# atoms-ufrj/atomsmm

Measured on AMD Instinct MI355X. Metric: ns/day on 100k-atom TIP3P RESPA box; near-nonbonded HBM GB/s vs 8 TB/s peak, higher is better.
Workload: dtype f64

## Files before the change

atomsmm_amd/csrc/abi.hip:

```cpp
#include <algorithm>
#include <cmath>
#include <cstring>
#include <numeric>

#include "amm_ctx.h"
#include "cluster.h"

int amm_pair_setup_grid(amm_ctx *ctx, PairForce *pf);
static bool amm_family_allows_cluster(int family, int flags) {
    const bool tab_family = family == AMM_NEAR_NONE || family == AMM_NEAR_SHIFT || family == AMM_NEAR_FSWITCH || family == AMM_DAMPED || family == AMM_NONBONDED;
    return tab_family && !(flags & (AMM_GROUP_LJ | AMM_GROUP_Q));
}
int amm_bonded_arity(int kind);
int amm_bonded_npar(int kind);

static thread_local std::string g_error;
void amm_set_error(const std::string &msg) { g_error = msg; }

static PairForce *get_pair(amm_ctx *ctx, int id) {
    if (!ctx || id < 0 || id >= (int)ctx->forces.size() || ctx->forces[id].type != AMM_FORCE_PAIR) {
        amm_set_error("invalid pair force id");
        return nullptr;
    }
    return ctx->forces[id].pair;
// ... 1208 lines not shown
    PairForce *pf = get_pair(ctx, force_id);
    if (!pf || !d_pos || !count) {
        amm_set_error("amm_pair_count_within: null argument or not a pair force");
        return 1;
    }
    if (pf->free_space) {
        amm_set_error("amm_pair_count_within: a free-space pair force (AMM_FREE_SPACE) has no neighbour rows to count");
        return 1;
    }
    long long c = 0;
    PairForce *Lw = pf->host ? pf->host : pf;
    if (Lw->last_kind >= 1 && Lw->cl && Lw->cl->built) {
        if (amm_cluster_count_within_impl(ctx, pf, d_pos, r_within, &c)) return 1;
        if (Lw->last_kind == 2 && pf->rest && Lw->rest && Lw->rest->built) {
            long long c2 = 0;
            if (amm_pair_count_within_impl(ctx, pf->rest, d_pos, r_within, &c2)) return 1;
            c += c2;
        }
    } else if (amm_pair_count_within_impl(ctx, pf, d_pos, r_within, &c)) return 1;
    *count = (int64_t)c;
    return 0;
}

const char *amm_kernel_revision(void) { return amm_kernel_revision_impl(); }

int amm_set_outer_skin(amm_ctx *ctx, double skin_out) {
    ctx->skin_out = skin_out;
    return 0;
}

int amm_set_option(amm_ctx *ctx, const char *name, double value) {
    if (!ctx || !name) {
        amm_set_error("amm_set_option: null argument");
        return 1;
    }
    const std::string k(name);
    const int v = (int)value;
    if (k == "cluster") ctx->opt_cluster = v;
    else if (k == "hybrid") ctx->opt_hybrid = v;
    else if (k == "small_group") ctx->opt_small_group = v;
    else if (k == "mixed_terms") ctx->opt_mixed_terms = v;
    else if (k == "rest_skin_factor") ctx->opt_rest_skin_factor = value;
    else if (k == "tab") ctx->opt_tab = v;
    else if (k == "site_trips") ctx->site_trips = v != 0;
    else if (k == "lanes_per_row") ctx->opt_lpa = v;
    else if (k == "build_parts") ctx->opt_parts = v;
    else if (k == "build_split") ctx->opt_build_split = v;
    else if (k == "unroll") ctx->opt_unroll = v;
    else if (k == "dual_unroll") ctx->opt_dual_unroll = v;
    else if (k == "tab_block") ctx->opt_tab_bs = v;
    else if (k == "tab_dual_block") ctx->opt_tab_dual_bs = v;
    else if (k == "fuse_rows") ctx->opt_fuse_rows = v;
    else if (k == "row_phases") ctx->opt_row_phases = v;
    else if (k == "group_candidates") ctx->opt_group_candidates = v;
    else if (k == "positions_private") ctx->opt_positions_private = v;
    else if (k == "site_tab") ctx->opt_site_tab = v;
    else if (k == "terms_from") ctx->opt_terms_from = v;
    else if (k == "no_term_lanes") ctx->opt_no_term_lanes = v;
    else if (k == "fuse_epilogue") ctx->opt_fuse_epilogue = v;
    else if (k == "comm_timeout") ctx->opt_comm_timeout = value;
    else if (k == "spec_assign") ctx->opt_spec_assign = v;
    else if (k == "chargeless") ctx->opt_chargeless = v;
    else if (k == "state_exchange") ctx->opt_state_exchange = v;
    else {
        amm_set_error("amm_set_option: unknown option '" + k + "'");
        return 1;
    }
    return 0;
}

static const double AMM_BOX_SKIN_KEEP = 0.5;
static const double AMM_BOX_ROWS_GROW = 1.25;

static double grid_room(const amm_ctx *ctx, const CellGrid &g) {
    double room = 1.0e30;
    for (int k = 0; k < 3; ++k) room = std::min(room, 2.0 * ctx->box.L[k] / g.nc[k]);
    return room;
}
static bool grid_differs(const amm_ctx *ctx, const CellGrid &g, double reach) {
    for (int k = 0; k < 3; ++k) {
        int nc = (int)floor(ctx->box.L[k] / (0.5 * reach));
        nc = std::max(1, std::min(512, nc));
        if (nc != g.nc[k]) return true;
    }
    return false;
}
static bool box_within(const amm_ctx *ctx, const double L0[3], double tol) {
    for (int k = 0; k < 3; ++k)
        if (std::fabs(ctx->box.L[k] - L0[k]) > tol * L0[k]) return false;
    return true;
}

static int box_apply(amm_ctx *ctx, bool &regrid, bool &waited) {
    const double V = ctx->box.L[0] * ctx->box.L[1] * ctx->box.L[2];
    for (auto &fo : ctx->forces) {
        if (fo.type != AMM_FORCE_PAIR || fo.pair->free_space) continue;
        PairForce *pf = fo.pair;
        pair_derive_buffers(ctx, pf);
        if (pf->rest) pf->rest->skin_req = pf->skin * ctx->opt_rest_skin_factor;
    }
    auto wait_once = [&]() -> int {
        if (!waited) AMM_HIP(hipStreamSynchronize(ctx->stream));
        waited = true;
        return 0;
    };
    for (auto &fo : ctx->forces) {
// ... 202 lines not shown
```

atomsmm_amd/csrc/amm_ctx.h:

```cpp
#pragma once
#include <hip/hip_runtime.h>

#include <cstdint>
#include <string>
#include <vector>

#include "../../include/atomsmm_hip.h"

#define AMM_WAVE 64
#define AMM_MAX_PRE 6
#define AMM_DERIV_LAMBDA 1024
#define AMM_MAX_GROUPS 33

void amm_set_error(const std::string &msg);
#define AMM_HIP(call)                                                                            \
    do {                                                                                         \
        hipError_t e_ = (call);                                                                  \
        if (e_ != hipSuccess) {                                                                  \
            amm_set_error(std::string(#call) + ": " + hipGetErrorString(e_));                    \
            return 1;                                                                            \
        }                                                                                        \
    } while (0)

struct PairTab {
// ... 244 lines not shown
#define AMM_MAX_WATCH 4
struct ListWatch {
    const double *xref = nullptr;
    double thr2 = 0;
    int *flags = nullptr;
    long *pre_epoch = nullptr;
    const double **pre_pos = nullptr;
};

static inline int amm_slice_per(int n, int world) {
    const int nc = (n + 2) / 3;
    return 3 * ((nc + world - 1) / world);
}

struct EpiPlan {
    BondedSet *bs = nullptr;
    double *f0 = nullptr;
    int npre = 0, niter = 0;
    const double *pre_a[AMM_MAX_PRE] = {nullptr}, *pre_b[AMM_MAX_PRE] = {nullptr};
    double pre_coef[AMM_MAX_PRE] = {0};
    int pre_plus[AMM_MAX_PRE] = {0};
    double c1 = 0, d = 0, c2 = 0;
    PairForce *next = nullptr;
    int kind = 0;
    int with_move = 0;
    double dcoef = 0;
};

struct amm_ctx {
    int n = 0;
    int opt_spec_assign = 1;
    int opt_state_exchange = 1;
    int opt_chargeless = 1;
    int opt_fuse_epilogue = 1;
    const EpiPlan *epi_request = nullptr;
    bool epi_done = false;
    long long n_epilogues = 0;
    long long n_state_exchanges = 0;
    std::vector<const double *> own_only;
    long long n_copies_current = 0;
    int opt_cluster = 1;
    int opt_hybrid = 1;
    double opt_rest_skin_factor = 2.0;
    int opt_mixed_terms = 1;
    int opt_small_group = 1;
    bool creating_rest = false;
    int opt_tab = 1;
    int opt_build_split = 0;
    int opt_lpa = 0, opt_parts = 0, opt_unroll = 2, opt_dual_unroll = 2, opt_tab_bs = 0, opt_tab_dual_bs = 0;
    int opt_site_tab = 1;
    CZeroRows zero_rows = CZeroRows{0, nullptr, nullptr, nullptr};
    int opt_positions_private = 0;
    int opt_group_candidates = 1;
    int opt_row_phases = 1;
    int opt_fuse_rows = 1;
    int opt_terms_from = 8192, opt_no_term_lanes = 0;
    ListWatch watched[AMM_MAX_WATCH];
    int n_watched = 0;
    int device = 0;
    hipStream_t stream = nullptr;
    Box box;
    bool has_box = true;
    int rank = 0, world = 1;
    std::vector<ForceObj> forces;
    double *d_x = nullptr, *d_v = nullptr;
    const double *d_mass = nullptr;
    double *slots[AMM_MAX_SLOTS] = {nullptr};
    GroupDef groups[AMM_MAX_GROUPS];
    bool profile = false;
    int profile_only = -1;
    double *d_scratch = nullptr;
    double *d_expr_part = nullptr;
    double *d_fscratch = nullptr;
    ConstraintSet *constraints = nullptr;
    std::vector<MinObj *> minimizers;
    std::vector<ExprDef> exprs;
    std::vector<BathDef> baths;
    IsoDef iso;
    RegDef reg;
    unsigned long long expr_seed = 0, expr_counter = 0;
    double *alt_x = nullptr, *alt_v = nullptr, *alt_f = nullptr;
    bool fuse_inner = true;
    bool site_trips = true;
    long long box_changes = 0, box_regrids = 0, box_waits = 0;
    int n_mol = 0, n_mol_small = 0, n_mol_long = 0;
    int *d_mol_ptr = nullptr, *d_mol_atoms = nullptr, *d_mol_small = nullptr, *d_mol_long = nullptr;
    long pos_epoch = 0;
    double skin_out = -1.0;
    void *comm = nullptr;
    bool comm_failed = false;
    double opt_comm_timeout = 0;
    double *d_xchg = nullptr;
    long long xchg_doubles = 0;
    PendingExchange pending;
    long long comm_calls = 0, comm_doubles = 0;
};

struct KickList {
    const double *f[4], *f2[4];
    int plus[4];
    double coef[4];
    int n;
};

#define AMM_FLAG_FAR 12
struct WatchArgs {
// ... 95 lines not shown
```

atomsmm_amd/csrc/cluster.hip:

```cpp
#include <algorithm>
#include <cmath>
#include <cstdio>
#include <cstdlib>
#include <cstring>
#include <type_traits>
#include <vector>

#include "amm_ctx.h"
#include "bonded_terms.h"
#include "cluster.h"
#include "device_utils.h"
#include "pair_math.h"
#include "pair_tab.h"

#ifndef AMM_EXP_NOLJ
#define AMM_EXP_NOLJ 0
#endif

__device__ double amm_erfcx_table_dev_c[AMM_ERFCX_NI * AMM_ERFCX_NC];
static bool g_erfcx_uploaded_c[64] = {false};

void amm_cluster_classify(int n, const std::vector<int> &ptr, const std::vector<int> &idx, std::vector<int> &mol_first, std::vector<int> &rest) {
    mol_first.clear();
    rest.clear();
// ... 828 lines not shown
                    }
                    row_cnt = lane == t ? (nf | (nb_ << 16)) : row_cnt;
                    j0 += nch;
                }
                CBS_STAMP(5);
                __syncthreads();
                CBS_STAMP(6);
            }
            if (w == 0 && lane < nt) {
                const int count = row_cnt & 0xffff, countf = (int)((unsigned)row_cnt >> 16);
                const int total_nb = count + countf;
                const bool over = total_nb > cap;
                nnb[tb + lane - c_begin] = over ? 0 : total_nb;
                nnb_near[tb + lane - c_begin] = over ? 0 : count;
                if (over) flags[1] = 1;
                wsum += (unsigned long long)total_nb;
                wnear += (unsigned long long)count;
                wmax = max(wmax, total_nb);
            }
        }
    }
    __syncthreads();
    }
    for (int off = 32; off > 0; off >>= 1) {
        wsum += __shfl_xor(wsum, off);
        wnear += __shfl_xor(wnear, off);
        wmax = max(wmax, __shfl_xor(wmax, off));
    }
    if (w == 0 && lane == 0) {
        amm_st_l2(&blockstats[3 * blockIdx.x], wsum);
        amm_st_l2(&blockstats[3 * blockIdx.x + 1], (unsigned long long)wmax);
        amm_st_l2(&blockstats[3 * blockIdx.x + 2], wnear);
    }
    if (amm_last_block(ticket)) cfinish_build_block(flags, counters, blockstats, (int)gridDim.x, 0);
}

#define AMM_CPHASES 6
struct CPairArgs {
    int c_begin, nrows, lpa_shift, cap;
    const int *aperm;
    const int *nl, *nnb, *nnb_total;
    const double4 *posq;
    const double2 *lj;
    double *force;
    int accumulate, sorted_out;
    Box box;
    const double *host_tab;
    int host_bytes;
    double margin;
    int ntask;
    int per_pair_image;
    int rpx, nphase;
    int ph_off[AMM_CPHASES], ph_shift[AMM_CPHASES], ph_ntask[AMM_CPHASES];
#ifdef AMM_CPAIR_TIMING
    unsigned long long *wave_times;
#endif
    const double *host_tab_ss;
    int host_ss_bytes, host_ss_off, site_atoms;
    double hsig_site, seps2_site;
    const double *guest_tab, *guest_tab_ss;
    int guest_bytes, guest_ss_bytes, guest_ss_off, g_accumulate;
    const double *tab_image;
    unsigned long long host_serial, guest_serial;
    PairForce *tab_owner;
    double *gforce;
    double gfac, gsr;
};

#ifdef AMM_CPAIR_TIMING
#define CWALK_T_PARAM , unsigned long long &t_first
#define CWALK_T_ARG , t_first
#else
#define CWALK_T_PARAM
#define CWALK_T_ARG
#endif
template <int FAM, int CMODE, int GFAM, int IMG, int SMASK>
__device__ __forceinline__ void cwalk_rows(const CPairArgs &A, const PairConsts &c, const PairConsts &g, const char *tabh, const char *tabg,
                                           const double *erfcx, const double4 (&pi)[3], const double2 *li, int i_sites, const int (&so)[3],
                                           const int (&sog)[3], double sign_lj, const int *row, int nfront, int nn, int sub, int lpa,
                                           int self, double (&f)[9], double (&fg)[9] CWALK_T_PARAM) {
    constexpr bool DUAL = GFAM >= 0;
    constexpr bool SS = SMASK != 0;
    const int back = A.cap - 1 + nfront;
    const double r2low = DUAL ? fmax(c.tab.r2min, g.tab.r2min) : c.tab.r2min;
    const double r2low_ss = DUAL ? fmax(c.tab.ss_r2min, g.tab.ss_r2min) : c.tab.ss_r2min;
    auto entry = [&](int k) { return k < nn ? row[k < nfront ? k : back - k] : self; };
    auto load_pos = [&](int e, int b) {
        return *reinterpret_cast<const double4 *>(reinterpret_cast<const char *>(A.posq) + (size_t)((unsigned)e & 0x1fffffffu) * 96u + 32 * b);
    };
    auto load_lj = [&](int e, int b) {
        double2 l = make_double2(0.0, 0.0);
        if (i_sites != 0 && __builtin_amdgcn_ballot_w64((((unsigned)e >> 29) >> b) & 1u) != 0ull)
            l = *reinterpret_cast<const double2 *>(reinterpret_cast<const char *>(A.lj) + (size_t)((unsigned)e & 0x1fffffffu) * 48u + 16 * b);
        return l;
    };
    double4 pj[3];
    double2 lj[3];
    int k = sub;
    int e = entry(k), en = entry(k + lpa);
#pragma unroll
    for (int b = 0; b < 3; ++b) {
        pj[b] = load_pos(e, b);
        if (!SS) lj[b] = load_lj(e, b);
    }
    while (__builtin_amdgcn_ballot_w64(k < nn) != 0ull) {
        const bool ok = k < nn;
        const bool front = k < nfront;
        const bool any_front = DUAL && __builtin_amdgcn_ballot_w64(front) != 0ull;
        const unsigned bits = (unsigned)e >> 29;
        const int e2 = entry(k + 2 * lpa);
        double sx = 0.0, sy = 0.0, sz = 0.0;
        if (IMG == 1) {
            sx = A.box.L[0] * rint((pj[0].x - pi[0].x) * A.box.invL[0]);
            sy = A.box.L[1] * rint((pj[0].y - pi[0].y) * A.box.invL[1]);
            sz = A.box.L[2] * rint((pj[0].z - pi[0].z) * A.box.invL[2]);
        }
#pragma unroll
        for (int b = 0; b < 3; ++b) {
            const double xb = pj[b].x - sx, yb = pj[b].y - sy, zb = pj[b].z - sz, qb = pj[b].w;
            const int mb = SS ? -(int)((bits >> b) & 1u) : 0;
// ... 402 lines not shown
    return all_most;
}

#ifndef AMM_CBS_SINGLE
#define AMM_CBS_SINGLE 512
#endif

#ifndef AMM_CBS_NEAR
#define AMM_CBS_NEAR 512
#endif
#ifndef AMM_CTAB_WAVES_PER_EU
#define AMM_CTAB_WAVES_PER_EU 1
#endif
template <int FAM, int CMODE, int GFAM, int BS, int SMASK, bool EPI = false>
__global__ void __launch_bounds__(BS) __attribute__((amdgpu_waves_per_eu(AMM_CTAB_WAVES_PER_EU)))
k_cpair(CPairArgs A, PairConsts c, PairConsts g, CEpiArgs E) {
    constexpr bool DUAL = GFAM >= 0;
    constexpr bool SS = SMASK != 0;
    extern __shared__ __align__(16) char s_lds[];
    if (EPI && E.spec_clear) {
        for (int cidx = blockIdx.x * BS + threadIdx.x; cidx <= E.grid.ncell; cidx += gridDim.x * BS) E.spec_clear[cidx] = 0;
    }
#ifdef AMM_CPAIR_TIMING
    const unsigned long long t_entry = wall_clock64();
    unsigned long long t_staged = 0, t_first = 0;
    int n_tasks_done = 0, n_interior = 0;
    unsigned long long t_epi[3] = {0, 0, 0};
#endif
    constexpr int WPB = BS / 64;
    const int lane = threadIdx.x & 63;
    const double sign = c.sign;
    const int xcd = blockIdx.x & 7, nwx = (gridDim.x >> 3) * WPB;
    const int row_end = min((xcd + 1) * A.rpx, A.nrows);
#ifdef AMM_CPAIR_SWAP
    const int wave = (int)(threadIdx.x >> 6) ^ 4;
#else
    const int wave = (int)(threadIdx.x >> 6);
#endif
    const int task0 = (int)(blockIdx.x >> 3) * WPB + __builtin_amdgcn_readfirstlane(wave);
    int phase = 0, task = task0;
    auto seek = [&]() {
        while (phase < A.nphase && task >= A.ph_ntask[phase]) {
            ++phase;
            task = task0;
        }
        return phase < A.nphase;
    };
    constexpr bool AHEAD = SS;
    int shift = 0, lpa = 1, sub = 0, a = 0, cs = 0, nfront = 0, nn = 0;
    bool valid = false;
    const int *row = nullptr;
    double4 pi[3];
    double2 pl[3];
    auto pre_rows = [&]() {
        shift = A.ph_shift[phase];
        lpa = 1 << shift;
        sub = lane & (lpa - 1);
        a = xcd * A.rpx + A.ph_off[phase] + task * (64 >> shift) + (lane >> shift);
        valid = a < row_end;
        cs = A.c_begin + (valid ? a : 0);
#pragma unroll
        for (int t = 0; t < 3; ++t) {
            pi[t] = A.posq[3 * cs + t];
            pl[t] = A.lj[3 * cs + t];
        }
        nfront = valid ? A.nnb[a] : 0;
        nn = valid ? (A.nnb_total ? A.nnb_total[a] : nfront) : 0;
        row = A.nl + (size_t)(valid ? a : 0) * A.cap;
    };
    bool has = seek();
    if (AHEAD && has) pre_rows();

    const int used = A.host_bytes + (DUAL ? A.guest_bytes : 0) + (SS ? A.host_ss_bytes + (DUAL ? A.guest_ss_bytes : 0) : 0);
    double2 tabs[(160 * 1024) / (BS * 16)];
    amm_stage_issue<BS>(tabs, A.tab_image, used);
    amm_stage_commit<BS>(tabs, s_lds, used);
    amm_stage_rest<BS>(tabs, A.tab_image, s_lds, used);
#if defined(AMM_EXP_TAB_GLOBAL)
    const char *tabh = reinterpret_cast<const char *>(A.host_tab);
#else
    const char *tabh = s_lds;
#endif
    const char *tabg = s_lds + A.host_bytes;
    const double *erfcx = amm_erfcx_table_dev_c;
    double2 *s_li = nullptr;
    if (!SS) {
        double *s_erfcx = reinterpret_cast<double *>(s_lds + used);
        for (int k = threadIdx.x; k < AMM_ERFCX_NI * AMM_ERFCX_NC; k += BS) s_erfcx[k] = amm_erfcx_table_dev_c[k];
        erfcx = s_erfcx;
        s_li = reinterpret_cast<double2 *>(s_erfcx + AMM_ERFCX_NI * AMM_ERFCX_NC) + (threadIdx.x >> 6) * 192;
    }
    __syncthreads();
#ifdef AMM_CPAIR_TIMING
    t_staged = wall_clock64();
#endif

    PairConsts c1 = c, g1 = g;
    c1.sign = 1.0;
    g1.sign = 1.0;
    while (has) {
        if (!AHEAD) pre_rows();
        const int t_a = a, t_cs = cs, t_sub = sub, t_lpa = lpa;
        const bool t_valid = valid;
        int i_sites = 0;
        int so[3] = {0, 0, 0}, sog[3] = {0, 0, 0};
        if (!SS) __builtin_amdgcn_wave_barrier();
#pragma unroll
        for (int t = 0; t < 3; ++t) {
            pi[t].w *= c.Kc * sign;
            double2 l = pl[t];
            l.y *= sign;
            if (!SS) s_li[64 * t + lane] = l;
            const bool site = valid && l.y != 0.0;
            if ((SMASK >> t) & 1) {
                so[t] = site ? A.host_ss_off : 0;
                if (DUAL) sog[t] = site ? A.guest_ss_off : 0;
            }
            if (__builtin_amdgcn_ballot_w64(site) != 0ull) i_sites |= 1 << t;
        }
        if (!SS) {
            __builtin_amdgcn_fence(__ATOMIC_RELEASE, "wavefront");
            __builtin_amdgcn_wave_barrier();
            __builtin_amdgcn_fence(__ATOMIC_ACQUIRE, "wavefront");
        }
        const double2 *li = SS ? nullptr : s_li + lane;
        const bool edge = valid && !(pi[0].x >= A.margin && pi[0].x <= A.box.L[0] - A.margin && pi[0].y >= A.margin &&
                                     pi[0].y <= A.box.L[1] - A.margin && pi[0].z >= A.margin && pi[0].z <= A.box.L[2] - A.margin);
        const bool interior = __builtin_amdgcn_ballot_w64(edge) == 0ull;
#ifdef AMM_CPAIR_TIMING
        ++n_tasks_done;
        n_interior += interior ? 1 : 0;
#endif
        double f[9], fg[9];
#pragma unroll
        for (int k = 0; k < 9; ++k) f[k] = fg[k] = 0.0;
        if (A.per_pair_image) cwalk_rows<FAM, CMODE, GFAM, 2, SMASK>(A, c1, g1, tabh, tabg, erfcx, pi, li, i_sites, so, sog, sign, row, nfront, nn, sub, lpa, cs, f, fg CWALK_T_ARG);
        else if (interior) cwalk_rows<FAM, CMODE, GFAM, 0, SMASK>(A, c1, g1, tabh, tabg, erfcx, pi, li, i_sites, so, sog, sign, row, nfront, nn, sub, lpa, cs, f, fg CWALK_T_ARG);
        else cwalk_rows<FAM, CMODE, GFAM, 1, SMASK>(A, c1, g1, tabh, tabg, erfcx, pi, li, i_sites, so, sog, sign, row, nfront, nn, sub, lpa, cs, f, fg CWALK_T_ARG);
        task += nwx;
        has = seek();
        if (AHEAD && has) pre_rows();
        for (int off = t_lpa >> 1; off > 0; off >>= 1) {
#pragma unroll
            for (int k = 0; k < 9; ++k) {
                f[k] += __shfl_xor(f[k], off);
                if (DUAL) fg[k] += __shfl_xor(fg[k], off);
            }
        }
        if (t_valid && t_sub == 0) {
#pragma unroll
            for (int t = 0; t < 3; ++t) {
                const int i = A.sorted_out ? 3 * t_a + t : A.aperm[3 * t_cs + t];
#pragma unroll
                for (int d = 0; d < 3; ++d) {
                    if (A.accumulate) A.force[3 * i + d] += f[3 * t + d];
                    else A.force[3 * i + d] = f[3 * t + d];
                    if (DUAL) {
                        if (A.g_accumulate) A.gforce[3 * i + d] += fg[3 * t + d];
                        else A.gforce[3 * i + d] = fg[3 * t + d];
                    }
                }
            }
        }
    }
#ifdef AMM_CPAIR_TIMING
    if (EPI) t_staged = wall_clock64();
#endif
    if (EPI) {
        for (int phase = 0; phase < A.nphase; ++phase) {
            const int shift = A.ph_shift[phase], row0 = xcd * A.rpx + A.ph_off[phase], ntask = A.ph_ntask[phase];
            const int rpw = 64 >> shift;
            for (int task = (int)(blockIdx.x >> 3) * WPB + (int)(threadIdx.x >> 6); task < ntask; task += nwx) {
                const int a = row0 + task * rpw + (lane >> shift);
                const bool valid = a < row_end;
#ifdef AMM_CPAIR_TIMING
                cepi_rows(E, A.box, A.c_begin + (valid ? a : 0), valid, lane & ((1 << shift) - 1), t_epi);
#else
                cepi_rows(E, A.box, A.c_begin + (valid ? a : 0), valid, lane & ((1 << shift) - 1));
#endif
            }
        }
        if (E.spec_count && amm_last_block(E.spec_ticket)) {
            if (amm_ld_l2(&E.spec_flags[0])) {
                const int fullest = cscan_counts<BS>(E.grid.ncell, E.spec_count, E.spec_start);
                if (threadIdx.x == 0) E.spec_flags[6] = fullest;
            }
        }
    }
#ifdef AMM_CPAIR_TIMING
    if (A.wave_times && (threadIdx.x & 63) == 0) {
        unsigned long long *o = A.wave_times + 4 * ((size_t)blockIdx.x * (BS / 64) + (threadIdx.x >> 6));
        o[0] = t_entry;
        o[1] = t_staged;
        o[2] = wall_clock64();
        o[3] = EPI ? (((t_epi[0] - t_staged) & 0xfffffull) | (((t_epi[1] - t_staged) & 0xfffffull) << 20) | (((t_epi[2] - t_staged) & 0xfffffull) << 40))
                   : ((((t_first ? t_first - t_entry : 0ull) & 0xfffffull) << 24) | ((unsigned long long)(n_interior & 0xffff) << 8) | (unsigned long long)(n_tasks_done & 0xff));
    }
#endif
}

static const double AMM_PHASE_COST[7] = {0, 0, 1.0, 0.55, 0.32, 0.18, 0.11};
static double cpair_plan_rec(int rows, int waves, int s, int off, CPairArgs *P) {
    const int rpw = 64 >> s, per_round = waves * rpw;
    const int full = rows / per_round, left = rows - full * per_round;
    const double finish = (double)((rows + per_round - 1) / per_round) * AMM_PHASE_COST[s];
    auto put = [&](int ntask) {
        if (P && ntask > 0) {
            P->ph_off[P->nphase] = off;
            P->ph_shift[P->nphase] = s;
            P->ph_ntask[P->nphase] = ntask;
            ++P->nphase;
        }
    };
    int s2 = 6;
    double split = 1e300;
    for (int t = s + 1; t <= 6 && left > 0; ++t) {
        const double v = cpair_plan_rec(left, waves, t, 0, nullptr);
        if (v < split) {
            split = v;
            s2 = t;
        }
    }
    split += full * AMM_PHASE_COST[s];
    if (left == 0 || s == 6 || finish <= split) {
        put((rows + rpw - 1) / rpw);
        return finish;
    }
    put(full * waves);
    cpair_plan_rec(left, waves, s2, off + full * per_round, P);
    return split;
}
static void cpair_plan(CPairArgs &P, int waves, int enabled) {
    P.rpx = (P.nrows + 7) / 8;
    P.nphase = 0;
    if (enabled) {
        cpair_plan_rec(P.rpx, waves, P.lpa_shift, 0, &P);
    } else {
        const int rpw = 64 >> P.lpa_shift;
        P.ph_off[0] = 0;
        P.ph_shift[0] = P.lpa_shift;
        P.ph_ntask[0] = (P.rpx + rpw - 1) / rpw;
        P.nphase = 1;
    }
}

static int cpair_tab_image(amm_ctx *ctx, CPairArgs &P, bool dual, bool ss) {
    const void *src[4] = {P.host_tab, dual ? P.guest_tab : nullptr, ss ? P.host_tab_ss : nullptr, (ss && dual) ? P.guest_tab_ss : nullptr};
    const int len[4] = {P.host_bytes, dual ? P.guest_bytes : 0, ss ? P.host_ss_bytes : 0, (ss && dual) ? P.guest_ss_bytes : 0};
    const unsigned long long gs = dual ? P.guest_serial : 0;
    const size_t bytes = (size_t)len[0] + len[1] + len[2] + len[3];
    PairForce::TabImage &im = P.tab_owner->tab_image[(dual ? 1 : 0) | (ss ? 2 : 0)];
    if (!(im.d && im.host_serial == P.host_serial && im.guest_serial == gs && im.bytes == bytes && im.stream == ctx->stream)) {
        im.host_serial = 0;
        if (im.d && im.stream != ctx->stream) AMM_HIP(hipDeviceSynchronize());
        if (im.bytes != bytes) {
            if (im.d) (void)hipFree(im.d);
            im.d = nullptr;
            im.bytes = 0;
            AMM_HIP(hipMalloc(&im.d, bytes));
            im.bytes = bytes;
        }
        size_t at = 0;
        for (int k = 0; k < 4; ++k) {
            if (len[k] > 0) AMM_HIP(hipMemcpyAsync(im.d + at, src[k], (size_t)len[k], hipMemcpyDeviceToDevice, ctx->stream));
            at += (size_t)len[k];
        }
        im.stream = ctx->stream;
        im.guest_serial = gs;
        im.host_serial = P.host_serial;
    }
    P.tab_image = reinterpret_cast<const double *>(im.d);
    return 0;
}

struct CLaunchCfg {
    int lds_set = 0, bpc = -1;
};
static int g_num_cu_c[64] = {0};

template <int FAM, int CMODE, int GFAM, int SMASK, bool EPI = false>
static int launch_cpair_t(amm_ctx *ctx, const CPairArgs &A, const PairConsts &c, const PairConsts &g, const CEpiArgs &E = CEpiArgs()) {
    constexpr bool DUAL = GFAM >= 0;
    constexpr int BS = DUAL ? AMM_CBS_SINGLE : AMM_CBS_NEAR;
    constexpr bool SS = SMASK != 0;
    static CLaunchCfg cfg[64];
    CLaunchCfg &k = cfg[ctx->device & 63];
    int lds = A.host_bytes + (DUAL ? A.guest_bytes : 0);
    if (SS) lds += A.host_ss_bytes + (DUAL ? A.guest_ss_bytes : 0);
    else lds += AMM_ERFCX_NI * AMM_ERFCX_NC * 8 + (BS / 64) * 192 * 16;
    auto kern = k_cpair<FAM, CMODE, GFAM, BS, SMASK, EPI>;
    if (lds > k.lds_set) {
        AMM_HIP(hipFuncSetAttribute(reinterpret_cast<const void *>(kern), hipFuncAttributeMaxDynamicSharedMemorySize, lds));
        k.lds_set = lds;
        k.bpc = -1;
    }
    if (k.bpc < 0) {
        int nb = 0;
        AMM_HIP(hipOccupancyMaxActiveBlocksPerMultiprocessor(&nb, kern, BS, (size_t)lds));
        if (nb < 1) {
            amm_set_error("molecule-row pair kernel does not fit on a CU (LDS)");
            return 1;
        }
        k.bpc = nb;
    }
    int &ncu = g_num_cu_c[ctx->device & 63];
    if (!ncu) AMM_HIP(hipDeviceGetAttribute(&ncu, hipDeviceAttributeMultiprocessorCount, ctx->device));
    constexpr int WPB = BS / 64;
    long nblk = std::min((long)ncu * k.bpc, ((long)A.ntask + WPB - 1) / WPB);
    nblk = std::max(8L, (nblk + 7) / 8 * 8);
    CPairArgs P = A;
    cpair_plan(P, (int)(nblk >> 3) * WPB, ctx->opt_row_phases);
    if (cpair_tab_image(ctx, P, DUAL, SS)) return 1;
#ifdef AMM_CPAIR_TIMING
    static int launches = 0;
    static unsigned long long *d_times = nullptr;
    const char *which = std::getenv("AMM_WAVE_TIMES");
    P.wave_times = nullptr;
    if (which && ++launches == std::atoi(which)) {
        const size_t nw = (size_t)nblk * WPB;
        AMM_HIP(hipMalloc(&d_times, sizeof(unsigned long long) * 4 * nw));
        P.wave_times = d_times;
        hipLaunchKernelGGL(kern, dim3((unsigned)nblk), dim3(BS), (size_t)lds, ctx->stream, P, c, g, E);
        std::vector<unsigned long long> h(4 * nw);
        AMM_HIP(hipMemcpy(h.data(), d_times, sizeof(unsigned long long) * 4 * nw, hipMemcpyDeviceToHost));
        std::string path = std::string(std::getenv("AMM_WAVE_TIMES_OUT") ? std::getenv("AMM_WAVE_TIMES_OUT") : "/tmp/wave_times") + (DUAL ? ".fused" : ".single") + (EPI ? "_epi" : "");
        if (FILE *fp = std::fopen(path.c_str(), "wb")) {
            std::fwrite(h.data(), sizeof(unsigned long long), h.size(), fp);
            std::fclose(fp);
        }
        return 0;
    }
#endif
    hipLaunchKernelGGL(kern, dim3((unsigned)nblk), dim3(BS), (size_t)lds, ctx->stream, P, c, g, E);
    return 0;
}

#define AMM_CPAIR_LDS_LIMIT (160 * 1024)
template <int FAM, int CMODE, int GFAM>
static int launch_cpair_s(amm_ctx *ctx, CPairArgs A, const PairConsts &c, const PairConsts &g, const CEpiArgs *E = nullptr, bool *epi_done = nullptr) {
    constexpr bool DUAL = GFAM >= 0;
    bool ss = ctx->opt_site_tab && A.host_ss_bytes > 0 && (!DUAL || A.guest_ss_bytes > 0);
    if (ss && A.host_bytes + A.host_ss_bytes + (DUAL ? A.guest_bytes + A.guest_ss_bytes : 0) > AMM_CPAIR_LDS_LIMIT) ss = false;
#ifndef AMM_CLUSTER_TUNE
    if (ss && E) {
        if (epi_done) *epi_done = true;
        return A.site_atoms == 1 ? launch_cpair_t<FAM, CMODE, GFAM, 1, true>(ctx, A, c, g, *E) : launch_cpair_t<FAM, CMODE, GFAM, 7, true>(ctx, A, c, g, *E);
    }
#endif
    if (ss) return A.site_atoms == 1 ? launch_cpair_t<FAM, CMODE, GFAM, 1>(ctx, A, c, g) : launch_cpair_t<FAM, CMODE, GFAM, 7>(ctx, A, c, g);
    PairConsts c0 = c, g0 = g;
    c0.tab.ss_first = g0.tab.ss_first = -1;
    A.host_ss_bytes = A.guest_ss_bytes = 0;
    return launch_cpair_t<FAM, CMODE, GFAM, 0>(ctx, A, c0, g0);
}

static int launch_cdual(amm_ctx *ctx, const CPairArgs &A, const PairConsts &c, const PairConsts &g, const CEpiArgs *E = nullptr, bool *epi_done = nullptr) {
    if (g.family != AMM_NEAR_FSWITCH) return -1;
    if (c.family == AMM_DAMPED && c.degree == 1) return launch_cpair_s<AMM_DAMPED, 1, AMM_NEAR_FSWITCH>(ctx, A, c, g, E, epi_done);
#ifndef AMM_CLUSTER_TUNE
    if (c.family == AMM_DAMPED) return launch_cpair_s<AMM_DAMPED, 0, AMM_NEAR_FSWITCH>(ctx, A, c, g, E, epi_done);
    if (c.family == AMM_NONBONDED) {
        if (c.cmode == 1) return launch_cpair_s<AMM_NONBONDED, 1, AMM_NEAR_FSWITCH>(ctx, A, c, g, E, epi_done);
        if (c.cmode == 2) return launch_cpair_s<AMM_NONBONDED, 2, AMM_NEAR_FSWITCH>(ctx, A, c, g, E, epi_done);
        return launch_cpair_s<AMM_NONBONDED, 0, AMM_NEAR_FSWITCH>(ctx, A, c, g, E, epi_done);
    }
#endif
    return -1;
}

static int launch_cpair(amm_ctx *ctx, const CPairArgs &A, const PairConsts &c, const CEpiArgs *E = nullptr, bool *epi_done = nullptr) {
#ifdef AMM_CLUSTER_TUNE
    if (c.family == AMM_NEAR_FSWITCH) return launch_cpair_s<AMM_NEAR_FSWITCH, 0, -1>(ctx, A, c, c);
    if (c.family == AMM_DAMPED && c.degree == 1) return launch_cpair_s<AMM_DAMPED, 1, -1>(ctx, A, c, c);
    amm_set_error("this is a kernel-tuning build (AMM_CLUSTER_TUNE): it holds the near force-switch and degree-1 damped kernels only");
    return 1;
#else
    switch (c.family) {
    case AMM_NEAR_NONE: return launch_cpair_s<AMM_NEAR_NONE, 0, -1>(ctx, A, c, c, E, epi_done);
    case AMM_NEAR_SHIFT: return launch_cpair_s<AMM_NEAR_SHIFT, 0, -1>(ctx, A, c, c, E, epi_done);
    case AMM_NEAR_FSWITCH: return launch_cpair_s<AMM_NEAR_FSWITCH, 0, -1>(ctx, A, c, c, E, epi_done);
    case AMM_DAMPED:
        if (c.degree == 1) return launch_cpair_s<AMM_DAMPED, 1, -1>(ctx, A, c, c, E, epi_done);
        return launch_cpair_s<AMM_DAMPED, 0, -1>(ctx, A, c, c, E, epi_done);
    default:
        if (c.cmode == 1) return launch_cpair_s<AMM_NONBONDED, 1, -1>(ctx, A, c, c, E, epi_done);
        if (c.cmode == 2) return launch_cpair_s<AMM_NONBONDED, 2, -1>(ctx, A, c, c, E, epi_done);
        return launch_cpair_s<AMM_NONBONDED, 0, -1>(ctx, A, c, c, E, epi_done);
    }
#endif
}
// ... 641 lines not shown
                       pf->d_seps2, pf->d_posq_s, pf->d_lj_s, (float)cl->rext, L->d_seps2, cl->d_first, CZeroRows{0, nullptr, nullptr, nullptr}, 0, (double *)nullptr, 0, 0, (int *)nullptr);
    if (cl->sorted_for == pf) {
        cl->sorted_epoch = ctx->pos_epoch;
        cl->sorted_pos = d_pos;
    }
    CPairArgs A;
    std::memset(&A, 0, sizeof(A));
    A.c_begin = cl->c_begin;
    A.nrows = cl->c_end - cl->c_begin;
    A.cap = cl->cap;
    A.nl = cl->d_nl;
    A.nnb = (pf == L) ? cl->d_nnb : cl->d_nnb_near;
    A.nnb_total = nullptr;
    if (pf == L && cl->rnear_build > 0) {
        A.nnb = cl->d_nnb_near;
        A.nnb_total = cl->d_nnb;
    }
    A.posq = pf->d_posq_s;
    A.box = ctx->box;
    unsigned long long *d_cnt = cl->d_counters + 7;
    AMM_HIP(hipMemsetAsync(d_cnt, 0, sizeof(unsigned long long), st));
    if (A.nrows > 0)
        hipLaunchKernelGGL(k_ccount_within, dim3((unsigned)(((long)A.nrows * 8 + 255) / 256)), dim3(256), 0, st, A, r_within * r_within, d_cnt);
    unsigned long long h = 0;
    AMM_HIP(hipMemcpyAsync(&h, d_cnt, sizeof(h), hipMemcpyDeviceToHost, st));
    AMM_HIP(hipStreamSynchronize(st));
    *count = (long long)h;
    return 0;
}

__global__ void __launch_bounds__(256) k_crow_padding(int nrows, int lpa_shift, const int *__restrict__ nnb, unsigned long long *out) {
    const int task = blockIdx.x * blockDim.x + threadIdx.x;
    const int rpw = 64 >> lpa_shift, lpa = 1 << lpa_shift;
    unsigned long long slots = 0, entries = 0;
    if (task * rpw < nrows) {
        int longest = 0;
        for (int r = task * rpw; r < min(nrows, (task + 1) * rpw); ++r) {
            const int nn = nnb[r];
            entries += (unsigned long long)nn;
            longest = max(longest, (nn + lpa - 1) >> lpa_shift);
        }
        slots = 64ull * (unsigned long long)longest;
    }
    for (int off = 32; off > 0; off >>= 1) {
        slots += __shfl_xor(slots, off);
        entries += __shfl_xor(entries, off);
    }
    if ((threadIdx.x & 63) == 0) {
        atomicAdd(&out[0], slots);
        atomicAdd(&out[1], entries);
    }
}

int amm_cluster_row_padding_impl(amm_ctx *ctx, PairForce *pf, long long out[2]) {
    PairForce *L = pf->host ? pf->host : pf;
    ClusterList *cl = L->cl;
    hipStream_t st = ctx->stream;
    const int nrows = cl->c_end - cl->c_begin;
    int sh = 0;
    while ((1 << sh) < cl->lpa) ++sh;
    unsigned long long *d_out = cl->d_counters + 5;
    AMM_HIP(hipMemsetAsync(d_out, 0, 2 * sizeof(unsigned long long), st));
    const int ntask = (nrows + (64 >> sh) - 1) / (64 >> sh);
    if (ntask > 0)
        hipLaunchKernelGGL(k_crow_padding, dim3((unsigned)((ntask + 255) / 256)), dim3(256), 0, st, nrows, sh, (pf == L) ? cl->d_nnb : cl->d_nnb_near, d_out);
    unsigned long long h[2] = {0, 0};
    AMM_HIP(hipMemcpyAsync(h, d_out, sizeof(h), hipMemcpyDeviceToHost, st));
    AMM_HIP(hipStreamSynchronize(st));
    out[0] = (long long)h[0];
    out[1] = (long long)h[1];
    return 0;
}

int amm_cluster_free(ClusterList *cl) {
#ifdef AMM_CBS_TIMING
    {
        unsigned long long t[8];
        const bool got = hipMemcpyFromSymbol(t, HIP_SYMBOL(g_cbs_t), sizeof(t)) == hipSuccess && t[7];
        if (got && cl->split_parts == 0)
            fprintf(stderr, "k_cbuild<SLICE>: %llu busy wavefronts, mean: prologue %.2f us, whole %.2f us, in drains %.2f us (%.2f drains)\n", t[7], t[0] / 100.0 / t[7],
                    t[1] / 100.0 / t[7], t[2] / 100.0 / t[7], (double)t[3] / t[7]);
        if (got && cl->split_parts > 0)
            fprintf(stderr, "k_cbuild_split, first wavefront of %llu busy blocks, mean clocks (100 MHz): prologue %.2f | pass 1 %.2f wait %.2f | pass 2 %.2f wait %.2f | copy %.2f wait %.2f us\n",
                    t[7], t[0] / 100.0 / t[7], t[1] / 100.0 / t[7], t[2] / 100.0 / t[7], t[3] / 100.0 / t[7], t[4] / 100.0 / t[7], t[5] / 100.0 / t[7], t[6] / 100.0 / t[7]);
    }
#endif
    for (void *q : {(void *)cl->d_spec_count[0], (void *)cl->d_spec_count[1], (void *)cl->d_spec_ticket})
        if (q) (void)hipFree(q);
    if (cl->d_slice_cells) (void)hipFree(cl->d_slice_cells);
    void *ptrs[] = {cl->d_cell_count, cl->d_cell_start, cl->d_cell_members, cl->d_cperm, cl->d_aperm, cl->d_pos4f, cl->d_xref, cl->d_nl,
                    cl->d_nnb, cl->d_nnb_near, cl->d_flags, cl->d_counters, cl->d_blockstats, cl->d_ticket};
    for (void *p : ptrs)
        if (p) (void)hipFree(p);
    delete cl;
    return 0;
}
```

atomsmm_amd/csrc/pair.hip:

```cpp
#include <atomic>
#include <cmath>
#include <cstdio>
#include <cstdlib>
#include <cstring>

#include "amm_ctx.h"
#include "bonded_terms.h"
#include "cluster.h"
#include "device_utils.h"
#include "pair_math.h"
#include "pair_tab.h"

int amm_pair_build_consts(const amm_pair_desc &d, PairConsts &pc) {
    pc.family = d.family;
    pc.flags = d.flags;
    pc.degree = d.degree < 1 ? 1 : d.degree;
    pc.cmode = (d.flags & AMM_COULOMB_EWALD) ? 1 : ((d.flags & AMM_COULOMB_RF) ? 2 : 0);
    pc.sign = d.sign;
    pc.rc = d.rc;
    pc.rc2 = d.rc * d.rc;
    pc.rc0 = d.rc0;
    pc.rs0 = d.rs0;
    pc.inv_dr0 = (d.rc0 > d.rs0) ? 1.0 / (d.rc0 - d.rs0) : 0.0;
    pc.rswitch = d.rswitch;
// ... 1928 lines not shown
        const int s = A.s_begin + a;
        const double4 pi = A.posq_s[s];
        const int nfront = A.nnb[a], nn = A.nnb_total ? A.nnb_total[a] : nfront;
        const int *row = A.nl + (size_t)a * A.cap;
        const int back = A.cap - 1 + nfront;
        for (int k = sub; k < nn; k += 1 << A.lpa_shift) {
            const double4 pj = A.posq_s[row[k < nfront ? k : back - k]];
            const double dx = amm_min_image(pi.x - pj.x, A.box.L[0], A.box.invL[0]);
            const double dy = amm_min_image(pi.y - pj.y, A.box.L[1], A.box.invL[1]);
            const double dz = amm_min_image(pi.z - pj.z, A.box.L[2], A.box.invL[2]);
            cnt += (dx * dx + dy * dy + dz * dz < r2w) ? 1ull : 0ull;
        }
    }
    for (int off = 32; off > 0; off >>= 1) cnt += __shfl_xor(cnt, off);
    if ((threadIdx.x & 63) == 0 && cnt) atomicAdd(out, cnt);
}

int amm_pair_count_within_impl(amm_ctx *ctx, PairForce *pf, const double *d_pos, double r_within, long long *count) {
    PairForce *L = pf->host ? pf->host : pf;
    if (!L->built) {
        amm_set_error("amm_pair_count_within: evaluate the force once first (the neighbour rows do not exist yet)");
        return 1;
    }
    hipStream_t st = ctx->stream;
    const int n = pf->n;
    hipLaunchKernelGGL(k_gather_sorted, dim3((n + 255) / 256), dim3(256), 0, st, n, L->d_perm, d_pos, pf->d_q, pf->d_hsig,
                       pf->d_seps2, ctx->box, pf->d_posq_s, pf->d_lj_s);
    PairArgs A;
    std::memset(&A, 0, sizeof(A));
    A.s_begin = L->s_begin;
    A.s_end = L->s_end;
    A.lpa_shift = 3;
    A.cap = L->cap;
    A.nl = L->d_nl;
    A.nnb = L->d_nnb_near;
    A.nnb_total = (pf == L && L->rnear_build > 0) ? L->d_nnb : nullptr;
    A.posq_s = pf->d_posq_s;
    A.box = ctx->box;
    const int nslice = L->s_end - L->s_begin;
    unsigned long long *d_cnt = L->d_counters + 7;
    AMM_HIP(hipMemsetAsync(d_cnt, 0, sizeof(unsigned long long), st));
    if (nslice > 0)
        hipLaunchKernelGGL(k_count_within, dim3((unsigned)(((long)nslice * 8 + 255) / 256)), dim3(256), 0, st, A, r_within * r_within, nslice, d_cnt);
    unsigned long long h = 0;
    AMM_HIP(hipMemcpyAsync(&h, d_cnt, sizeof(h), hipMemcpyDeviceToHost, st));
    AMM_HIP(hipStreamSynchronize(st));
    *count = (long long)h;
    return 0;
}

extern "C" __attribute__((weak)) const char *amm_variant_tag(void);
const char *amm_kernel_revision_impl() {
#ifdef AMM_CLUSTER_TUNE
    return "r06-prologue-tune";
#else
    return amm_variant_tag ? "r06-prologue-tune" : "r06-prologue";
#endif
}

int amm_pair_build_table(PairForce *pf) {
    std::vector<double> coef;
    SiteTable ss;
    ss.want = pf->cluster_ok && pf->one_site_class && pf->site_one_charge && pf->site_q != 0.0 && pf->site_seps2 != 0.0;
    ss.sig = 2.0 * pf->site_hsig;
    ss.eps4 = pf->site_seps2 * pf->site_seps2;
    ss.QQ = pf->pc.Kc * pf->site_q * pf->site_q;
    pf->tab_error = amm_build_coulomb_table(pf->pc, coef, &ss);
    pf->ss_built_for[0] = pf->site_hsig;
    pf->ss_built_for[1] = pf->site_seps2;
    pf->ss_built_for[2] = ss.want ? pf->site_q : 0.0;
    if (pf->d_tab) {
        (void)hipFree(pf->d_tab);
        pf->d_tab = nullptr;
    }
    if (pf->d_tab_ss) {
        (void)hipFree(pf->d_tab_ss);
        pf->d_tab_ss = nullptr;
    }
    pf->ss_error = ss.error;
    static std::atomic<unsigned long long> uploads{0};
    pf->tab_serial = ++uploads;
    if (pf->pc.tab.nint > 0 && !(pf->tab_error <= AMM_TAB_MAX_ERROR)) {
        pf->pc.tab.nint = 0;
        coef.clear();
    }
    if (pf->pc.tab.nint == 0 || ss.coef.empty() || !(ss.error <= AMM_TAB_SS_MAX_ERROR)) {
        pf->pc.tab.ss_first = -1;
        ss.coef.clear();
    }
    if (pf->pc.tab.nint > 0) {
        AMM_HIP(hipMalloc(&pf->d_tab, sizeof(double) * coef.size()));
        AMM_HIP(hipMemcpy(pf->d_tab, coef.data(), sizeof(double) * coef.size(), hipMemcpyHostToDevice));
    }
    if (!ss.coef.empty()) {
        AMM_HIP(hipMalloc(&pf->d_tab_ss, sizeof(double) * ss.coef.size()));
        AMM_HIP(hipMemcpy(pf->d_tab_ss, ss.coef.data(), sizeof(double) * ss.coef.size(), hipMemcpyHostToDevice));
    }
    return 0;
}

bool amm_pair_can_fuse_discount(amm_ctx *ctx, PairForce *guest, PairForce *host) {
    if (!guest || !host || guest->host != host || host->host) return false;
    if (!(guest->desc.flags & AMM_GUARD_RC0)) return false;
    if (guest->fuse_ok >= 0) return guest->fuse_ok == 1;
    guest->fuse_ok = 0;
    if (!ctx->opt_tab) return false;
    const int gf = guest->desc.family, hf = host->desc.family;
    if (!(gf == AMM_NEAR_NONE || gf == AMM_NEAR_SHIFT || gf == AMM_NEAR_FSWITCH)) return false;
    if (!(hf == AMM_DAMPED || hf == AMM_NONBONDED)) return false;
// ... 67 lines not shown
```

Baseline: 1097.

## Deal cluster rows to wavefronts by sorted cost within each block

When the pair kernel runs a single phase with at most one task per wave, each block now computes a cost key per row window (neighbor count, dual guest work, and whether the cluster sits near the box edge). It ranks these keys in LDS and reassigns rows so that rows of similar cost share a wavefront. This is meant to cut divergence and padding from mixing long and short neighbor rows in one wave. The change costs extra LDS, two block barriers and a prologue load per launch, and the row-padding diagnostic is updated to report on the dealt assignment.

```diff
diff --git a/atomsmm_amd/csrc/abi.hip b/atomsmm_amd/csrc/abi.hip
--- a/atomsmm_amd/csrc/abi.hip
+++ b/atomsmm_amd/csrc/abi.hip
@@ -1284,6 +1284,7 @@
     else if (k == "tab_dual_block") ctx->opt_tab_dual_bs = v;
     else if (k == "fuse_rows") ctx->opt_fuse_rows = v;
     else if (k == "row_phases") ctx->opt_row_phases = v;
+    else if (k == "deal_rows") ctx->opt_deal_rows = v;
     else if (k == "group_candidates") ctx->opt_group_candidates = v;
     else if (k == "positions_private") ctx->opt_positions_private = v;
     else if (k == "site_tab") ctx->opt_site_tab = v;
diff --git a/atomsmm_amd/csrc/amm_ctx.h b/atomsmm_amd/csrc/amm_ctx.h
--- a/atomsmm_amd/csrc/amm_ctx.h
+++ b/atomsmm_amd/csrc/amm_ctx.h
@@ -320,6 +320,7 @@
     CZeroRows zero_rows = CZeroRows{0, nullptr, nullptr, nullptr};
     int opt_positions_private = 0;
     int opt_group_candidates = 1;
+    int opt_deal_rows = 1;
     int opt_row_phases = 1;
     int opt_fuse_rows = 1;
     int opt_terms_from = 8192, opt_no_term_lanes = 0;
diff --git a/atomsmm_amd/csrc/cluster.hip b/atomsmm_amd/csrc/cluster.hip
--- a/atomsmm_amd/csrc/cluster.hip
+++ b/atomsmm_amd/csrc/cluster.hip
@@ -904,6 +904,7 @@
     int per_pair_image;
     int rpx, nphase;
     int ph_off[AMM_CPHASES], ph_shift[AMM_CPHASES], ph_ntask[AMM_CPHASES];
+    int deal_off;
 #ifdef AMM_CPAIR_TIMING
     unsigned long long *wave_times;
 #endif
@@ -918,6 +919,40 @@
     double *gforce;
     double gfac, gsr;
 };
+
+#define AMM_DEAL_UNIT 8
+#define AMM_DEAL_GUEST 7
+__host__ __device__ inline unsigned cdeal_key(bool valid, bool edge, int nfront, int nn, int shift, bool dual, int idx) {
+    const int lpa = 1 << shift;
+    int cost = AMM_DEAL_UNIT * ((nn + lpa - 1) >> shift) + (dual ? AMM_DEAL_GUEST * ((nfront + lpa - 1) >> shift) : 0);
+    cost = cost < 0x1fffff ? cost : 0x1fffff;
+    return valid ? ((edge ? 1u << 30 : 0u) | ((unsigned)cost << 9) | (unsigned)idx) : (0x80000000u | (unsigned)idx);
+}
+__host__ __device__ inline bool cdeal_edge(double x, double y, double z, const Box &box, double margin) {
+    return !(x >= margin && x <= box.L[0] - margin && y >= margin && y <= box.L[1] - margin && z >= margin && z <= box.L[2] - margin);
+}
+__host__ __device__ inline int cdeal_group(int wave, int wpb) { return (wpb == 8 && wave >= 4) ? 11 - wave : wave; }
+static inline int cdeal_bytes(int bs, int shift) { return (6 * (bs >> shift) + 15) & ~15; }
+static inline bool cdeal_applies(int enabled, int nphase, const int *ph_ntask, int waves_per_xcd) {
+    return enabled && nphase == 1 && ph_ntask[0] <= waves_per_xcd;
+}
+template <int BS>
+__device__ __forceinline__ void cdeal_rank(unsigned key, int shift, char *lds) {
+    unsigned *keys = reinterpret_cast<unsigned *>(lds);
+    unsigned short *map = reinterpret_cast<unsigned short *>(lds + 4 * (BS >> shift));
+    const int lpa = 1 << shift, sub = (int)threadIdx.x & (lpa - 1), wrow = (int)threadIdx.x >> shift, nwin = BS >> shift;
+    if (sub == 0) keys[wrow] = key;
+    __syncthreads();
+    int rank = 0;
+    for (int j = sub; j < nwin; j += lpa) rank += keys[j] < key ? 1 : 0;
+    for (int off = lpa >> 1; off > 0; off >>= 1) rank += __shfl_xor(rank, off);
+    if (sub == 0) map[rank] = (unsigned short)wrow;
+    __syncthreads();
+}
+__device__ __forceinline__ int cdeal_row(const char *lds, int bs, int shift, int wave, int lane) {
+    const unsigned short *map = reinterpret_cast<const unsigned short *>(lds + 4 * (bs >> shift));
+    return (int)map[cdeal_group(wave, bs >> 6) * (64 >> shift) + (lane >> shift)];
+}
 
 #ifdef AMM_CPAIR_TIMING
 #define CWALK_T_PARAM , unsigned long long &t_first
@@ -1426,11 +1461,11 @@
     const int *row = nullptr;
     double4 pi[3];
     double2 pl[3];
-    auto pre_rows = [&]() {
+    auto pre_rows = [&](int wrow) {
         shift = A.ph_shift[phase];
         lpa = 1 << shift;
         sub = lane & (lpa - 1);
-        a = xcd * A.rpx + A.ph_off[phase] + task * (64 >> shift) + (lane >> shift);
+        a = xcd * A.rpx + A.ph_off[phase] + wrow;
         valid = a < row_end;
         cs = A.c_begin + (valid ? a : 0);
 #pragma unroll
@@ -1442,12 +1477,31 @@
         nn = valid ? (A.nnb_total ? A.nnb_total[a] : nfront) : 0;
         row = A.nl + (size_t)(valid ? a : 0) * A.cap;
     };
+    auto own_rows = [&]() { return task * (64 >> A.ph_shift[phase]) + (lane >> A.ph_shift[phase]); };
     bool has = seek();
-    if (AHEAD && has) pre_rows();
+    const bool deal = A.deal_off != 0;
+    const int win0 = (int)(blockIdx.x >> 3) * (BS >> A.ph_shift[0]);
+    unsigned dkey = 0;
+    if (deal) {
+        const int dshift = A.ph_shift[0], wrow = (int)threadIdx.x >> dshift;
+        const int a0 = xcd * A.rpx + A.ph_off[0] + win0 + wrow;
+        const bool v0 = a0 < row_end;
+        const int nf0 = A.nnb[v0 ? a0 : 0], nt0 = A.nnb_total ? A.nnb_total[v0 ? a0 : 0] : nf0;
+        const double4 p0 = A.posq[3 * (A.c_begin + (v0 ? a0 : 0))];
+        dkey = cdeal_key(v0, cdeal_edge(p0.x, p0.y, p0.z, A.box, A.margin), nf0, nt0, dshift, DUAL, wrow);
+    } else if (AHEAD && has) pre_rows(own_rows());
 
     const int used = A.host_bytes + (DUAL ? A.guest_bytes : 0) + (SS ? A.host_ss_bytes + (DUAL ? A.guest_ss_bytes : 0) : 0);
     double2 tabs[(160 * 1024) / (BS * 16)];
     amm_stage_issue<BS>(tabs, A.tab_image, used);
+    if (deal) {
+        cdeal_rank<BS>(dkey, A.ph_shift[0], s_lds + A.deal_off);
+        const int wrow = win0 + cdeal_row(s_lds + A.deal_off, BS, A.ph_shift[0], wave, lane);
+        phase = 0;
+        task = task0;
+        has = __builtin_amdgcn_readfirstlane(xcd * A.rpx + A.ph_off[0] + wrow) < row_end;
+        if (AHEAD && has) pre_rows(wrow);
+    }
     amm_stage_commit<BS>(tabs, s_lds, used);
     amm_stage_rest<BS>(tabs, A.tab_image, s_lds, used);
 #if defined(AMM_EXP_TAB_GLOBAL)
@@ -1473,7 +1527,7 @@
     c1.sign = 1.0;
     g1.sign = 1.0;
     while (has) {
-        if (!AHEAD) pre_rows();
+        if (!AHEAD) pre_rows(deal ? win0 + cdeal_row(s_lds + A.deal_off, BS, A.ph_shift[0], wave, lane) : own_rows());
         const int t_a = a, t_cs = cs, t_sub = sub, t_lpa = lpa;
         const bool t_valid = valid;
         int i_sites = 0;
@@ -1513,7 +1567,7 @@
         else cwalk_rows<FAM, CMODE, GFAM, 1, SMASK>(A, c1, g1, tabh, tabg, erfcx, pi, li, i_sites, so, sog, sign, row, nfront, nn, sub, lpa, cs, f, fg CWALK_T_ARG);
         task += nwx;
         has = seek();
-        if (AHEAD && has) pre_rows();
+        if (AHEAD && has) pre_rows(own_rows());
         for (int off = t_lpa >> 1; off > 0; off >>= 1) {
 #pragma unroll
             for (int k = 0; k < 9; ++k) {
@@ -1544,8 +1598,13 @@
         for (int phase = 0; phase < A.nphase; ++phase) {
             const int shift = A.ph_shift[phase], row0 = xcd * A.rpx + A.ph_off[phase], ntask = A.ph_ntask[phase];
             const int rpw = 64 >> shift;
-            for (int task = (int)(blockIdx.x >> 3) * WPB + (int)(threadIdx.x >> 6); task < ntask; task += nwx) {
-                const int a = row0 + task * rpw + (lane >> shift);
+            int task = (int)(blockIdx.x >> 3) * WPB + (int)(threadIdx.x >> 6), drow = 0;
+            if (deal) {
+                drow = win0 + cdeal_row(s_lds + A.deal_off, BS, shift, wave, lane);
+                task = __builtin_amdgcn_readfirstlane(row0 + drow) < row_end ? 0 : ntask;
+            }
+            for (; task < ntask; task += nwx) {
+                const int a = row0 + (deal ? drow : task * rpw + (lane >> shift));
                 const bool valid = a < row_end;
 #ifdef AMM_CPAIR_TIMING
                 cepi_rows(E, A.box, A.c_begin + (valid ? a : 0), valid, lane & ((1 << shift) - 1), t_epi);
@@ -1647,8 +1706,9 @@
     return 0;
 }
 
+#define AMM_CPAIR_LDS_LIMIT (160 * 1024)
 struct CLaunchCfg {
-    int lds_set = 0, bpc = -1;
+    int lds_set = 0, bpc = -1, deal_set = 0;
 };
 static int g_num_cu_c[64] = {0};
 
@@ -1664,7 +1724,7 @@
     else lds += AMM_ERFCX_NI * AMM_ERFCX_NC * 8 + (BS / 64) * 192 * 16;
     auto kern = k_cpair<FAM, CMODE, GFAM, BS, SMASK, EPI>;
     if (lds > k.lds_set) {
-        AMM_HIP(hipFuncSetAttribute(reinterpret_cast<const void *>(kern), hipFuncAttributeMaxDynamicSharedMemorySize, lds));
+        AMM_HIP(hipFuncSetAttribute(reinterpret_cast<const void *>(kern), hipFuncAttributeMaxDynamicSharedMemorySize, std::max(lds, k.deal_set)));
         k.lds_set = lds;
         k.bpc = -1;
     }
@@ -1684,6 +1744,18 @@
     nblk = std::max(8L, (nblk + 7) / 8 * 8);
     CPairArgs P = A;
     cpair_plan(P, (int)(nblk >> 3) * WPB, ctx->opt_row_phases);
+    P.deal_off = 0;
+    {
+        const int off = (lds + 15) & ~15, need = off + cdeal_bytes(BS, P.ph_shift[0]);
+        if (cdeal_applies(ctx->opt_deal_rows, P.nphase, P.ph_ntask, (int)(nblk >> 3) * WPB) && need + 256 <= AMM_CPAIR_LDS_LIMIT) {
+            if (need > std::max(k.lds_set, k.deal_set)) {
+                AMM_HIP(hipFuncSetAttribute(reinterpret_cast<const void *>(kern), hipFuncAttributeMaxDynamicSharedMemorySize, need));
+                k.deal_set = need;
+            }
+            P.deal_off = off;
+            lds = need;
+        }
+    }
     if (cpair_tab_image(ctx, P, DUAL, SS)) return 1;
 #ifdef AMM_CPAIR_TIMING
     static int launches = 0;
@@ -1709,7 +1781,6 @@
     return 0;
 }
 
-#define AMM_CPAIR_LDS_LIMIT (160 * 1024)
 template <int FAM, int CMODE, int GFAM>
 static int launch_cpair_s(amm_ctx *ctx, CPairArgs A, const PairConsts &c, const PairConsts &g, const CEpiArgs *E = nullptr, bool *epi_done = nullptr) {
     constexpr bool DUAL = GFAM >= 0;
@@ -2457,6 +2528,52 @@
     }
 }
 
+template <int BS>
+__global__ void __launch_bounds__(BS) k_crow_padding_dealt(int nrows, int c_begin, int shift, int rpx, const int *__restrict__ nfront_of,
+                                                           const int *__restrict__ nn_of, const double4 *__restrict__ posq, Box box, double margin,
+                                                           int dual, int deal, unsigned long long *out) {
+    __shared__ __align__(16) char s_map[6 * BS + 16];
+    const int xcd = blockIdx.x & 7, lane = threadIdx.x & 63, wave = (int)(threadIdx.x >> 6);
+    const int row_end = min((xcd + 1) * rpx, nrows), win0 = (int)(blockIdx.x >> 3) * (BS >> shift);
+    const int wrow = (int)threadIdx.x >> shift, a0 = xcd * rpx + win0 + wrow;
+    const bool v0 = a0 < row_end;
+    const double4 p0 = posq[3 * (c_begin + (v0 ? a0 : 0))];
+    if (deal) cdeal_rank<BS>(cdeal_key(v0, cdeal_edge(p0.x, p0.y, p0.z, box, margin), nfront_of[v0 ? a0 : 0], nn_of[v0 ? a0 : 0], shift, dual != 0, wrow), shift, s_map);
+    const int a = deal ? xcd * rpx + win0 + cdeal_row(s_map, BS, shift, wave, lane) : a0;
+    const int nn = a < row_end ? nn_of[a] : 0;
+    int longest = (nn + (1 << shift) - 1) >> shift;
+    unsigned long long entries = (lane & ((1 << shift) - 1)) == 0 ? (unsigned long long)nn : 0ull;
+    for (int off = 32; off > 0; off >>= 1) {
+        longest = max(longest, __shfl_xor(longest, off));
+        entries += __shfl_xor(entries, off);
+    }
+    if (lane == 0 && entries) {
+        atomicAdd(&out[0], 64ull * (unsigned long long)longest);
+        atomicAdd(&out[1], entries);
+    }
+}
+
+template <int BS>
+static int crow_padding_dealt(amm_ctx *ctx, PairForce *pf, ClusterList *cl, int sh, bool dual, unsigned long long *d_out, int *dealt) {
+    constexpr int WPB = BS / 64;
+    const int nrows = cl->c_end - cl->c_begin, ntask = (nrows + (64 >> sh) - 1) / (64 >> sh);
+    int &ncu = g_num_cu_c[ctx->device & 63];
+    if (!ncu) AMM_HIP(hipDeviceGetAttribute(&ncu, hipDeviceAttributeMultiprocessorCount, ctx->device));
+    long nblk = std::min((long)ncu, ((long)ntask + WPB - 1) / WPB);
+    nblk = std::max(8L, (nblk + 7) / 8 * 8);
+    CPairArgs P;
+    std::memset(&P, 0, sizeof(P));
+    P.nrows = nrows;
+    P.lpa_shift = sh;
+    cpair_plan(P, (int)(nblk >> 3) * WPB, ctx->opt_row_phases);
+    *dealt = cdeal_applies(1, P.nphase, P.ph_ntask, (int)(nblk >> 3) * WPB) ? 1 : 0;
+    if (*dealt)
+        hipLaunchKernelGGL(k_crow_padding_dealt<BS>, dim3((unsigned)nblk), dim3(BS), 0, ctx->stream, nrows, cl->c_begin, P.ph_shift[0], P.rpx, cl->d_nnb_near,
+                           pf->host ? cl->d_nnb_near : cl->d_nnb, pf->d_posq_s, ctx->box,
+                           cl->rlist_build + cl->skin + 2.0 * cl->rext + 1e-6, dual ? 1 : 0, ctx->opt_deal_rows ? 1 : 0, d_out);
+    return 0;
+}
+
 int amm_cluster_row_padding_impl(amm_ctx *ctx, PairForce *pf, long long out[2]) {
     PairForce *L = pf->host ? pf->host : pf;
     ClusterList *cl = L->cl;
@@ -2467,7 +2584,11 @@
     unsigned long long *d_out = cl->d_counters + 5;
     AMM_HIP(hipMemsetAsync(d_out, 0, 2 * sizeof(unsigned long long), st));
     const int ntask = (nrows + (64 >> sh) - 1) / (64 >> sh);
-    if (ntask > 0)
+    const bool dual = pf == L && cl->rnear_build > 0;
+    int dealt = 0;
+    if (ntask > 0 && (dual ? crow_padding_dealt<AMM_CBS_SINGLE>(ctx, pf, cl, sh, dual, d_out, &dealt) : crow_padding_dealt<AMM_CBS_NEAR>(ctx, pf, cl, sh, dual, d_out, &dealt)))
+        return 1;
+    if (ntask > 0 && !dealt)
         hipLaunchKernelGGL(k_crow_padding, dim3((unsigned)((ntask + 255) / 256)), dim3(256), 0, st, nrows, sh, (pf == L) ? cl->d_nnb : cl->d_nnb_near, d_out);
     unsigned long long h[2] = {0, 0};
     AMM_HIP(hipMemcpyAsync(h, d_out, sizeof(h), hipMemcpyDeviceToHost, st));
diff --git a/atomsmm_amd/csrc/pair.hip b/atomsmm_amd/csrc/pair.hip
--- a/atomsmm_amd/csrc/pair.hip
+++ b/atomsmm_amd/csrc/pair.hip
@@ -2004,9 +2004,9 @@
 extern "C" __attribute__((weak)) const char *amm_variant_tag(void);
 const char *amm_kernel_revision_impl() {
 #ifdef AMM_CLUSTER_TUNE
-    return "r06-prologue-tune";
+    return "r07-deal-tune";
 #else
-    return amm_variant_tag ? "r06-prologue-tune" : "r06-prologue";
+    return amm_variant_tag ? "r07-deal-tune" : "r07-deal";
 #endif
 }
 
```

Measured after the change: 1090. No clear change (-0.6%).
